# metatensor/metatrain

Hardware: AMD Instinct MI355X
Metric: atom-steps/sec (energy+forces) PET 10k-atom box (higher is better)
Workload: dtype f32; 1 GPU; PET forward + dE/dR (preprocess+features+predict+backward), 8 x 10000-atom boxes per GPU per step, default PET hypers (2.9M params), 4.5 A cutoff, 191050 edges/box; parallelism=boxes sharded over 1 rank(s), no data-path collective

## Files before the change

metatrain_amd/csrc/rows_s.h:

```cpp
#pragma once
#include "ablk.h"

namespace pet {

constexpr int RING_NW = 4;
constexpr size_t RING_LDS_BYTES = RING_NW * 16384 + RING_NSLOT * RING_SLOT;

#define RING_WAVE(R)                                                                              \
    extern __shared__ __attribute__((aligned(16))) char ring_smem[];                             \
    const RowLane L;                                                                              \
    const unsigned lane16 = (unsigned)L.lane * 16u;                                               \
    const int wave = __builtin_amdgcn_readfirstlane(threadIdx.x >> 6);                            \
    int64_t row0 = ((int64_t)blockIdx.x * RING_NW + wave) * WROWS;                                \
    const bool live = row0 < (R);                                                                 \
    if (!live) row0 = (((R) - 1) / WROWS) * WROWS;                                                \
    [[maybe_unused]] const int64_t row = row0 + L.r < (R) ? row0 + L.r : (R) - 1;                 \
    [[maybe_unused]] const bool valid = live && row0 + L.r < (R);                                 \
    char* tile = ring_smem + wave * 16384;                                                        \
    const char* ring = ring_smem + RING_NW * 16384;                                               \
    const unsigned tile_u = __builtin_amdgcn_readfirstlane((unsigned)(uintptr_t)tile);            \
    const unsigned ring_u = __builtin_amdgcn_readfirstlane((unsigned)(uintptr_t)ring)
#define RING_SLOT_DST(ring_u, wave, g) ((ring_u) + (unsigned)((g) & (RING_NSLOT - 1)) * RING_SLOT + (wave) * 1024)
#define RING_SLOT_PTR(ring, g, lane16) ((ring) + ((g) & (RING_NSLOT - 1)) * RING_SLOT + (lane16))
__device__ __forceinline__ int ring_clamp(int g, int n) { return g < n ? g : n - 1; }
template <int SPC, int NC>
__device__ __forceinline__ void ring_clamp_chunk(int& hc, int& s) {
    if (s >= SPC) { s -= SPC; hc += 1; }
    if (hc >= NC) { hc = NC - 1; s = SPC - 1; }
}

template <int EXTRA = 0>
__device__ __forceinline__ void ring_stage_sync(bool extra_in_flight = false, bool drain = false) {
    if (extra_in_flight && drain) asm volatile("s_waitcnt vmcnt(0) lgkmcnt(0)" ::: "memory");
    else if (extra_in_flight) asm volatile("s_waitcnt vmcnt(%0) lgkmcnt(0)" ::"n"(2 + EXTRA) : "memory");
    else asm volatile("s_waitcnt vmcnt(2) lgkmcnt(0)" ::: "memory");
#ifndef AB_ABL_NOBAR
    __syncthreads();
#endif
}

__device__ __forceinline__ void ring_stage_mfma(const char* slot, f32x16& a0, const f16x8& x0h, const f16x8& x0l, f32x16& a1,
                                                const f16x8& x1h, const f16x8& x1l) {
    const f16x8 w0h = *reinterpret_cast<const f16x8*>(slot);
    const f16x8 w0l = *reinterpret_cast<const f16x8*>(slot + 1024);
    AB_MFMA3(a0, w0h, w0l, x0h, x0l);
    const f16x8 w1h = *reinterpret_cast<const f16x8*>(slot + 2048);
    const f16x8 w1l = *reinterpret_cast<const f16x8*>(slot + 3072);
    AB_MFMA3(a1, w1h, w1l, x1h, x1l);
}

template <int LEAD = 0, int NT = 4, int KB = 8, class Req>
__device__ __forceinline__ void hs_gemm_r(f32x16 (&acc)[NT], const f16x8 (&xh)[KB], const f16x8 (&xl)[KB], int g0, Req req,
                                          const char* ring, unsigned lane16, bool lead = false) {
#pragma unroll
    for (int r = 0; r < (NT / 2) * KB; r++) {
        const int g = g0 + r, tp = r / KB, kb = r % KB;
        if (r < 3 && lead) ring_stage_sync<LEAD>(true);
        else ring_stage_sync();
        req(g + 3);
        ring_stage_mfma(RING_SLOT_PTR(ring, g, lane16), acc[2 * tp], xh[kb], xl[kb], acc[2 * tp + 1], xh[kb], xl[kb]);
    }
}
template <int KB>
__device__ __forceinline__ void hs_planes(const float4 (&x)[2 * KB], f16x8 (&xh)[KB], f16x8 (&xl)[KB], float f = ABS) {
#pragma unroll
    for (int kb = 0; kb < KB; kb++) {
        const float v8[8] = {x[2 * kb].x * f, x[2 * kb].y * f, x[2 * kb].z * f, x[2 * kb].w * f,
                             x[2 * kb + 1].x * f, x[2 * kb + 1].y * f, x[2 * kb + 1].z * f, x[2 * kb + 1].w * f};
        ab_split8(v8, xh[kb], xl[kb]);
    }
}
__device__ __forceinline__ float hs_vec(const float* __restrict__ v, int t, int j, int i, int h) {
    const float lo = v[32 * t + 8 * j + i], hi = v[32 * t + 8 * j + 4 + i];
    return h ? hi : lo;
}
__device__ __forceinline__ float hs_vec_s(const float* __restrict__ v, int t, int j, int i, int h) {
    const float lo = ab_sload(v + 32 * t + 8 * j + i), hi = ab_sload(v + 32 * t + 8 * j + 4 + i);
    return h ? hi : lo;
}
template <int NT>
__device__ __forceinline__ void hs_acc_rows(float4 (&y)[4 * NT], const f32x16* acc, float f, const float* __restrict__ bias = nullptr,
                                            int off = 0, int h = 0) {
#pragma unroll
    for (int t = 0; t < NT; t++)
#pragma unroll
        for (int j = 0; j < 4; j++) {
            const f32x16& a = acc[t];
            y[4 * t + j] = make_float4(a[4 * j] * f, a[4 * j + 1] * f, a[4 * j + 2] * f, a[4 * j + 3] * f);
            if (bias) {
                y[4 * t + j].x += hs_vec(bias + off, t, j, 0, h); y[4 * t + j].y += hs_vec(bias + off, t, j, 1, h);
                y[4 * t + j].z += hs_vec(bias + off, t, j, 2, h); y[4 * t + j].w += hs_vec(bias + off, t, j, 3, h);
            }
        }
}

__device__ __forceinline__ void ring_dma_rows(const float* __restrict__ X, int64_t r0, int64_t R, int ld, unsigned lds_base,
                                              const RowLane& L) {
    const float* base = X + r0 * ld;
    const int rmax = (int)(R - 1 - r0 < 31 ? R - 1 - r0 : 31);
    const int hi = L.lane >> 5, c = L.lane & 31;
#pragma unroll
    for (int j = 0; j < 16; j++) {
        const int r = 2 * j + hi, rr = r < rmax ? r : rmax;
        const unsigned off = ((unsigned)rr * (unsigned)ld + 4u * (unsigned)(c ^ (r & 15))) * 4u;
        unsigned keep;
        asm volatile("s_mov_b32 %0, m0\n\ts_mov_b32 m0, %3\n\ts_nop 0\n\tglobal_load_lds_dwordx4 %1, %2\n\ts_mov_b32 m0, %0"
                     : "=&s"(keep) : "v"(off), "s"(base), "s"(lds_base + j * 1024) : "memory");
    }
}

inline W2 lin_planes(const void* planes, const Lin& l) { return w2_planes(planes, l.n_out / 32, l.k_in / 16); }
template <class... P, class... A>
inline void launch_ring(void (*kern)(P...), int64_t rows, hipStream_t st, A... args) {
    allow_big_lds(kern, RING_LDS_BYTES);
    kern<<<cdiv(rows, RING_NW * WROWS), 256, RING_LDS_BYTES, st>>>(static_cast<P>(args)...);
}

}
```

metatrain_amd/csrc/so_rows_s.hip:

```cpp
#include "rows_s.h"
#include "tile.h"

namespace pet {

__device__ __forceinline__ float rs_pick(const float* __restrict__ v, int i, int h) { return h ? v[i + 4] : v[i]; }

__global__ __launch_bounds__(256, 2) void k_rowgemm_s(const float* __restrict__ X, int ldx, int nk, const float* __restrict__ cs,
                                                     W2 w, const float* __restrict__ bias, float* __restrict__ Y, int ldy, int nn,
                                                     int64_t R, const float* __restrict__ A ) {
    RING_WAVE(R);
    const int kbt = 8 * nk, np = nk * nn;
    const f16x8* plane = (wave & 1) ? w.l : w.h;
    auto piece = [=](int nb, int ks, int s, int g) {
        const unsigned dst = RING_SLOT_DST(ring_u, wave, g);
        ab_dma_piece(plane, (4 * nb + 2 * (s >> 3) + (wave >> 1)) * kbt + 8 * ks + (s & 7), lane16, dst);
    };
    ring_dma_rows(X, row0, R, ldx, tile_u, L);
    piece(0, 0, 0, 0);
    piece(0, 0, 1, 1);
    piece(0, 0, 2, 2);
    asm volatile("s_waitcnt vmcnt(3)" ::: "memory");
    f16x8 xh[8], xl[8];
    f32x16 acc[4];
    float scale = 0.f, inv = 0.f;
#pragma unroll 1
    for (int p = 0; p < np; p++) {
        const int nb = __builtin_amdgcn_readfirstlane(p / nk), ks = __builtin_amdgcn_readfirstlane(p - nb * nk);
        bool lead = nk == 1 && nb > 0;
        RowLane Lp = L;
        asm volatile("" : "+v"(Lp.lane), "+v"(Lp.r), "+v"(Lp.h));
        int64_t r0 = row0;
        asm volatile("" : "+s"(r0));
        if (ks == 0) {
#pragma unroll
            for (int t = 0; t < 4; t++) acc[t] = ab_zero();
        }
        if (nk > 1 || p == 0) {
            float4 x[16];
            tile128_to_frag(x, tile, Lp);
            if (cs) {
                const float* v = cs + 128 * ks;
#pragma unroll
                for (int kg = 0; kg < 16; kg++) {
                    x[kg].x *= rs_pick(v, 8 * kg + 0, Lp.h);
                    x[kg].y *= rs_pick(v, 8 * kg + 1, Lp.h);
                    x[kg].z *= rs_pick(v, 8 * kg + 2, Lp.h);
                    x[kg].w *= rs_pick(v, 8 * kg + 3, Lp.h);
                }
            }
            float sc;
            const float iv = row_pow2<16>(x, sc);
            const bool shrink = ks == 0 || sc < scale;
            const float sc_eff = shrink ? sc : scale;
            if (ks > 0) {
                const float f = sc_eff * inv;
#pragma unroll
                for (int t = 0; t < 4; t++)
#pragma unroll
                    for (int i = 0; i < 16; i++) acc[t][i] *= f;
            }
            scale = sc_eff;
            inv = shrink ? iv : inv;
#pragma unroll
            for (int kg = 0; kg < 16; kg++) { x[kg].x *= sc_eff; x[kg].y *= sc_eff; x[kg].z *= sc_eff; x[kg].w *= sc_eff; }
            hs_planes(x, xh, xl);
        }
        if (ks + 1 < nk) {
            asm volatile("s_waitcnt lgkmcnt(0)" ::: "memory");
            __builtin_amdgcn_wave_barrier();
            ring_dma_rows(X + 128 * (ks + 1), r0, R, ldx, tile_u, Lp);
            lead = true;
        }
        {
            const bool last = p + 1 == np;
            const int ksn = ks + 1 < nk ? ks + 1 : 0, nbn = ks + 1 < nk ? nb : nb + 1;
            hs_gemm_r<16>(acc, xh, xl, 0, [=](int s) {
                if (s < 16) piece(nb, ks, s, s);
                else if (last) piece(nb, ks, 15, s);
                else piece(nbn, ksn, s - 16, s);
            }, ring, lane16, lead);
        }
        if (ks + 1 < nk) continue;
        const float f = inv * ABQ_INV;
        const float* bv = bias ? bias + 128 * nb : nullptr;
#pragma unroll
        for (int g = 0; g < 2; g++) {
            float4 y[8];
#pragma unroll
            for (int t = 0; t < 2; t++)
#pragma unroll
                for (int j = 0; j < 4; j++) {
                    const f32x16& a = acc[2 * g + t];
                    y[4 * t + j] = make_float4(a[4 * j] * f, a[4 * j + 1] * f, a[4 * j + 2] * f, a[4 * j + 3] * f);
                }
            if (bv) {
                const float* v = bv + 64 * g;
#pragma unroll
                for (int kg = 0; kg < 8; kg++) {
                    y[kg].x += rs_pick(v, 8 * kg + 0, Lp.h);
                    y[kg].y += rs_pick(v, 8 * kg + 1, Lp.h);
                    y[kg].z += rs_pick(v, 8 * kg + 2, Lp.h);
                    y[kg].w += rs_pick(v, 8 * kg + 3, Lp.h);
                }
            }
            const int col = 128 * nb + 64 * g;
            int64_t r0 = row0;
            asm volatile("" : "+s"(r0));
            auto out = [&](int r) { return live && r0 + r < R ? Y + (r0 + r) * ldy + col : nullptr; };
            __builtin_amdgcn_wave_barrier();
            if (A) {
                float4 old[8];
                request_rows_addend<8>(old, Lp, [&](int r) { return A + (r0 + r < R ? r0 + r : R - 1) * ldy + col; });
                store_rows_lines_add<8>(y, old, reinterpret_cast<float*>(tile), Lp, out);
            } else
                store_rows_lines<8>(y, reinterpret_cast<float*>(tile), Lp, out);
        }
        if (nk > 1 && nb + 1 < nn) {
            asm volatile("s_waitcnt lgkmcnt(0)" ::: "memory");
            __builtin_amdgcn_wave_barrier();
            int64_t r1 = row0;
            asm volatile("" : "+s"(r1));
            ring_dma_rows(X, r1, R, ldx, tile_u, Lp);
            asm volatile("s_waitcnt vmcnt(0)" ::: "memory");
        }
    }
}


#define RS_SETUP() \
    RING_WAVE(R);  \
    const f16x8* plane = (wave & 1) ? w.l : w.h
#define RS_LANE(Lx)                            \
    RowLane Lx = L;                            \
    asm volatile("" : "+v"(Lx.lane));          \
    Lx.r = Lx.lane & 31;                       \
    Lx.h = Lx.lane >> 5
#define RS_ROW0(rx) int64_t rx = row0; asm volatile("" : "+s"(rx))

__device__ __forceinline__ void rs_store_block(const f32x16 (&acc)[4], float f, const float* __restrict__ bv, const float* __restrict__ A,
                                               float* __restrict__ Y, int ldy, int col, int64_t r0, int64_t R, bool live, char* tile,
                                               const RowLane& Lq) {
    const int64_t row = r0 + Lq.r < R ? r0 + Lq.r : R - 1;
#pragma unroll
    for (int t = 0; t < 4; t++) {
        float4 y[4];
#pragma unroll
        for (int j = 0; j < 4; j++) y[j] = make_float4(acc[t][4 * j] * f, acc[t][4 * j + 1] * f, acc[t][4 * j + 2] * f, acc[t][4 * j + 3] * f);
        if (bv) {
#pragma unroll
            for (int j = 0; j < 4; j++) {
                const float4 b4 = *reinterpret_cast<const float4*>(bv + 32 * t + 8 * j + 4 * Lq.h);
                y[j].x += b4.x; y[j].y += b4.y; y[j].z += b4.z; y[j].w += b4.w;
            }
        }
        if (A) {
            float4 a4[4];
            load_rowfrag<4>(a4, A + col + 32 * t, row, ldy, Lq.h);
#pragma unroll
            for (int j = 0; j < 4; j++) { y[j].x += a4[j].x; y[j].y += a4[j].y; y[j].z += a4[j].z; y[j].w += a4[j].w; }
        }
        __builtin_amdgcn_wave_barrier();
        store_tile32_lines(y, reinterpret_cast<float*>(tile), Y + col + 32 * t, r0, live ? R : 0, ldy, Lq);
    }
}

__device__ __forceinline__ void rs_store_block_swiglu_bwd(const f32x16 (&acc)[4], float f, const float* __restrict__ VG,
                                                          float* __restrict__ dVG, int hid, int col, int64_t r0, int64_t R, bool live,
                                                          char* tile, const RowLane& Lq) {
    const int64_t row = r0 + Lq.r < R ? r0 + Lq.r : R - 1;
#pragma unroll
    for (int t = 0; t < 4; t++) {
        float4 v4[4], g4[4], dv[4], dg[4];
        load_rowfrag<4>(v4, VG + col + 32 * t, row, 2 * hid, Lq.h);
        load_rowfrag<4>(g4, VG + hid + col + 32 * t, row, 2 * hid, Lq.h);
#pragma unroll
        for (int j = 0; j < 4; j++) {
            const float du[4] = {acc[t][4 * j] * f, acc[t][4 * j + 1] * f, acc[t][4 * j + 2] * f, acc[t][4 * j + 3] * f};
            const float sx = sigmoidf_(g4[j].x), sy = sigmoidf_(g4[j].y), sz = sigmoidf_(g4[j].z), sw = sigmoidf_(g4[j].w);
            dv[j] = make_float4(du[0] * sx, du[1] * sy, du[2] * sz, du[3] * sw);
            dg[j] = make_float4(du[0] * v4[j].x * sx * (1.f - sx), du[1] * v4[j].y * sy * (1.f - sy), du[2] * v4[j].z * sz * (1.f - sz),
                                du[3] * v4[j].w * sw * (1.f - sw));
        }
        __builtin_amdgcn_wave_barrier();
        store_tile32_lines(dv, reinterpret_cast<float*>(tile), dVG + col + 32 * t, r0, live ? R : 0, 2 * hid, Lq);
        store_tile32_lines(dg, reinterpret_cast<float*>(tile), dVG + hid + col + 32 * t, r0, live ? R : 0, 2 * hid, Lq);
    }
}
__device__ __forceinline__ void rs_store_norm_bwd(f32x16 (&a0)[4], f32x16 (&a1)[4], float f, const float* __restrict__ x,
                                                  const float* __restrict__ gamma, int ln, const float* __restrict__ dres,
                                                  float* __restrict__ out, int64_t r0, int64_t R, bool live, char* tile,
                                                  const RowLane& Lq) {
    const int64_t row = r0 + Lq.r < R ? r0 + Lq.r : R - 1;
    float s1 = 0.f, s2 = 0.f, sx = 0.f, sxx = 0.f;
#pragma unroll
    for (int b = 0; b < 2; b++)
#pragma unroll
        for (int t = 0; t < 4; t++) {
            f32x16& a = b ? a1[t] : a0[t];
            float4 x4[4];
            load_rowfrag<4>(x4, x + 128 * b + 32 * t, row, 256, Lq.h);
#pragma unroll
            for (int j = 0; j < 4; j++) {
                const float4 g = *reinterpret_cast<const float4*>(gamma + 128 * b + 32 * t + 8 * j + 4 * Lq.h);
                const float xv[4] = {x4[j].x, x4[j].y, x4[j].z, x4[j].w}, gv[4] = {g.x, g.y, g.z, g.w};
#pragma unroll
                for (int i = 0; i < 4; i++) {
                    const float d = a[4 * j + i] * f * gv[i];
                    a[4 * j + i] = d;
                    s1 += d; s2 = fmaf(d, xv[i], s2); sx += xv[i]; sxx = fmaf(xv[i], xv[i], sxx);
                }
            }
        }
    s1 = row_sum(s1); s2 = row_sum(s2); sx = row_sum(sx); sxx = row_sum(sxx);
    const float mean = ln ? sx * (1.0f / 256.0f) : 0.f;
    const float var = sxx * (1.0f / 256.0f) - mean * mean;
    const float rstd = rsqrtf(var + (ln ? 1e-5f : 1.1920928955078125e-07f));
    const float m1 = ln ? s1 * (1.0f / 256.0f) : 0.f;
    const float m2 = (s2 - mean * s1) * rstd * (1.0f / 256.0f);
#pragma unroll
    for (int b = 0; b < 2; b++)
#pragma unroll
        for (int t = 0; t < 4; t++) {
            const f32x16& a = b ? a1[t] : a0[t];
            float4 x4[4], r4[4], y[4];
            load_rowfrag<4>(x4, x + 128 * b + 32 * t, row, 256, Lq.h);
            load_rowfrag<4>(r4, dres + 128 * b + 32 * t, row, 256, Lq.h);
#pragma unroll
            for (int j = 0; j < 4; j++)
                y[j] = make_float4(r4[j].x + rstd * (a[4 * j] - m1 - (x4[j].x - mean) * rstd * m2),
                                   r4[j].y + rstd * (a[4 * j + 1] - m1 - (x4[j].y - mean) * rstd * m2),
                                   r4[j].z + rstd * (a[4 * j + 2] - m1 - (x4[j].z - mean) * rstd * m2),
                                   r4[j].w + rstd * (a[4 * j + 3] - m1 - (x4[j].w - mean) * rstd * m2));
            __builtin_amdgcn_wave_barrier();
            store_tile32_lines(y, reinterpret_cast<float*>(tile), out + 128 * b + 32 * t, r0, live ? R : 0, 256, Lq);
        }
}

template <int NORM, int EPI = 0>
__global__ __launch_bounds__(256, 2) void k_rowgemm_s_k2(const float* __restrict__ X, int ldx, const float* __restrict__ cs,
                                                        const float* __restrict__ cb, W2 w, const float* __restrict__ bias,
                                                        const float* __restrict__ A, float* __restrict__ Y, int ldy, int nn, int64_t R) {
    RS_SETUP();
    const bool full = live && row0 + WROWS <= R;
    constexpr int nk = 2, kbt = 16;
    auto piece = [=](int nb, int ks, int s, int g) {
        const unsigned dst = RING_SLOT_DST(ring_u, wave, g);
        ab_dma_piece(plane, (4 * nb + 2 * (s >> 3) + (wave >> 1)) * kbt + 8 * ks + (s & 7), lane16, dst);
    };
    ring_dma_rows(X, row0, R, ldx, tile_u, L);
    asm volatile("s_waitcnt vmcnt(0)" ::: "memory");
    f16x8 xh[2][8], xl[2][8];
    float inv;
    {
        float4 x0[16], x1[16];
        tile128_to_frag(x0, tile, L);
        asm volatile("s_waitcnt lgkmcnt(0)" ::: "memory");
        __builtin_amdgcn_wave_barrier();
        ring_dma_rows(X + 128, row0, R, ldx, tile_u, L);
        asm volatile("s_waitcnt vmcnt(0)" ::: "memory");
        tile128_to_frag(x1, tile, L);
        if (NORM) {
            float mean = 0.f;
            if (NORM == 2) {
                float s1 = 0.f;
#pragma unroll
                for (int k = 0; k < 16; k++) s1 += (x0[k].x + x0[k].y) + (x0[k].z + x0[k].w) + (x1[k].x + x1[k].y) + (x1[k].z + x1[k].w);
                mean = row_sum(s1) * (1.0f / 256.0f);
            }
            float s2 = 0.f;
#pragma unroll
            for (int k = 0; k < 16; k++) {
                if (NORM == 2) {
                    x0[k].x -= mean; x0[k].y -= mean; x0[k].z -= mean; x0[k].w -= mean;
                    x1[k].x -= mean; x1[k].y -= mean; x1[k].z -= mean; x1[k].w -= mean;
                }
                s2 += x0[k].x * x0[k].x + x0[k].y * x0[k].y + x0[k].z * x0[k].z + x0[k].w * x0[k].w;
                s2 += x1[k].x * x1[k].x + x1[k].y * x1[k].y + x1[k].z * x1[k].z + x1[k].w * x1[k].w;
            }
            const float rstd = rsqrtf(row_sum(s2) * (1.0f / 256.0f) + (NORM == 2 ? 1e-5f : 1.1920928955078125e-07f));
#pragma unroll
            for (int k = 0; k < 16; k++) {
                const float4 g0 = *reinterpret_cast<const float4*>(cs + 8 * k + 4 * L.h);
                const float4 g1 = *reinterpret_cast<const float4*>(cs + 128 + 8 * k + 4 * L.h);
                x0[k] = make_float4(x0[k].x * rstd * g0.x, x0[k].y * rstd * g0.y, x0[k].z * rstd * g0.z, x0[k].w * rstd * g0.w);
                x1[k] = make_float4(x1[k].x * rstd * g1.x, x1[k].y * rstd * g1.y, x1[k].z * rstd * g1.z, x1[k].w * rstd * g1.w);
                if (NORM == 2) {
                    const float4 b0 = *reinterpret_cast<const float4*>(cb + 8 * k + 4 * L.h);
                    const float4 b1 = *reinterpret_cast<const float4*>(cb + 128 + 8 * k + 4 * L.h);
                    x0[k].x += b0.x; x0[k].y += b0.y; x0[k].z += b0.z; x0[k].w += b0.w;
                    x1[k].x += b1.x; x1[k].y += b1.y; x1[k].z += b1.z; x1[k].w += b1.w;
                }
            }
        } else if (cs) {
#pragma unroll
            for (int k = 0; k < 16; k++) {
                const float4 g0 = *reinterpret_cast<const float4*>(cs + 8 * k + 4 * L.h);
                const float4 g1 = *reinterpret_cast<const float4*>(cs + 128 + 8 * k + 4 * L.h);
                x0[k].x *= g0.x; x0[k].y *= g0.y; x0[k].z *= g0.z; x0[k].w *= g0.w;
                x1[k].x *= g1.x; x1[k].y *= g1.y; x1[k].z *= g1.z; x1[k].w *= g1.w;
            }
        }
        float sc0, sc1;
        const float iv0 = row_pow2<16>(x0, sc0), iv1 = row_pow2<16>(x1, sc1);
        const float sc = sc0 < sc1 ? sc0 : sc1;
        inv = sc0 < sc1 ? iv0 : iv1;
#pragma unroll
        for (int k = 0; k < 16; k++) { x0[k].x *= sc; x0[k].y *= sc; x0[k].z *= sc; x0[k].w *= sc; }
        hs_planes(x0, xh[0], xl[0]);
#pragma unroll
        for (int k = 0; k < 16; k++) { x1[k].x *= sc; x1[k].y *= sc; x1[k].z *= sc; x1[k].w *= sc; }
        hs_planes(x1, xh[1], xl[1]);
    }
    asm volatile("s_waitcnt vmcnt(0) lgkmcnt(0)" ::: "memory");
    piece(0, 0, 0, 0);
    piece(0, 0, 1, 1);
    piece(0, 0, 2, 2);
    const float f = inv * ABQ_INV;
#pragma unroll 1
    for (int nb = 0; nb < nn; nb++) {
        f32x16 acc[4];
#pragma unroll
        for (int t = 0; t < 4; t++) acc[t] = ab_zero();
        const bool last = nb + 1 == nn;
        if (nb > 0 && !full) asm volatile("s_waitcnt vmcnt(0)" ::: "memory");
        if (EPI == 1 && nb > 0) asm volatile("s_waitcnt vmcnt(0)" ::: "memory");
        hs_gemm_r<16>(acc, xh[0], xl[0], 0, [=](int s) {
            if (s < 16) piece(nb, 0, s, s); else piece(nb, 1, s - 16, s);
        }, ring, lane16, EPI == 0 && nb > 0 && full);
        hs_gemm_r(acc, xh[1], xl[1], 0, [=](int s) {
            if (s < 16) piece(nb, 1, s, s);
            else if (last) piece(nb, 1, 15, s);
            else piece(nb + 1, 0, s - 16, s);
        }, ring, lane16);
        RS_LANE(Lq);
        RS_ROW0(r0);
        if (EPI == 1) rs_store_block_swiglu_bwd(acc, f, A, Y, 128 * nn, 128 * nb, r0, R, live, tile, Lq);
        else rs_store_block(acc, f, bias ? bias + 128 * nb : nullptr, A, Y, ldy, 128 * nb, r0, R, live, tile, Lq);
    }
}

template <int EPI = 0>
__global__ __launch_bounds__(256, 2) void k_rowgemm_s_n2(const float* __restrict__ X, int ldx, int nk, W2 w,
                                                        const float* __restrict__ bias, const float* __restrict__ A,
                                                        float* __restrict__ Y, int ldy, int64_t R,
                                                        const float* __restrict__ xn = nullptr, int ln = 0) {
    RS_SETUP();
    const int kbt = 8 * nk;
    auto piece = [=](int nb, int ks, int s, int g) {
        const unsigned dst = RING_SLOT_DST(ring_u, wave, g);
        ab_dma_piece(plane, (4 * nb + 2 * (s >> 3) + (wave >> 1)) * kbt + 8 * ks + (s & 7), lane16, dst);
    };
    ring_dma_rows(X, row0, R, ldx, tile_u, L);
    piece(0, 0, 0, 0);
    piece(0, 0, 1, 1);
    piece(0, 0, 2, 2);
    asm volatile("s_waitcnt vmcnt(3)" ::: "memory");
    f32x16 acc0[4], acc1[4];
#pragma unroll
    for (int t = 0; t < 4; t++) { acc0[t] = ab_zero(); acc1[t] = ab_zero(); }
    f16x8 xh[8], xl[8];
    float scale = 0.f, inv = 0.f;
#pragma unroll 1
    for (int ks = 0; ks < nk; ks++) {
        RS_LANE(Lp);
        RS_ROW0(r0);
        {
            const char* rowp = tile + 512 * Lp.r;
            const int sw = Lp.r & 15;
            float m = 0.f;
#pragma unroll
            for (int kg = 0; kg < 16; kg++) {
                const float4 v = *reinterpret_cast<const float4*>(rowp + 16 * ((2 * kg + Lp.h) ^ sw));
                m = fmaxf(fmaxf(m, fmaxf(fabsf(v.x), fabsf(v.y))), fmaxf(fabsf(v.z), fabsf(v.w)));
            }
            m = fmaxf(m, __shfl_xor(m, 32));
            int e = (__float_as_int(m) >> 23) & 0xff;
            e = e > 253 ? 253 : e;
            const float sc = __int_as_float((254 - e) << 23), iv = __int_as_float(e << 23);
            const bool shrink = ks == 0 || sc < scale;
            const float sc_eff = shrink ? sc : scale;
            if (ks > 0) {
                const float g = sc_eff * inv;
#pragma unroll
                for (int t = 0; t < 4; t++)
#pragma unroll
                    for (int i = 0; i < 16; i++) { acc0[t][i] *= g; acc1[t][i] *= g; }
            }
            scale = sc_eff;
            inv = shrink ? iv : inv;
            const float fs = sc_eff;
#pragma unroll
            for (int kb = 0; kb < 8; kb++) {
                const float4 a = *reinterpret_cast<const float4*>(rowp + 16 * ((4 * kb + Lp.h) ^ sw));
                const float4 b = *reinterpret_cast<const float4*>(rowp + 16 * ((4 * kb + 2 + Lp.h) ^ sw));
                const float v8[8] = {a.x * fs * ABS, a.y * fs * ABS, a.z * fs * ABS, a.w * fs * ABS,
                                     b.x * fs * ABS, b.y * fs * ABS, b.z * fs * ABS, b.w * fs * ABS};
                ab_split8(v8, xh[kb], xl[kb]);
            }
        }
        const bool more = ks + 1 < nk;
        if (more) {
            asm volatile("s_waitcnt lgkmcnt(0)" ::: "memory");
            __builtin_amdgcn_wave_barrier();
            ring_dma_rows(X + 128 * (ks + 1), r0, R, ldx, tile_u, Lp);
        }
        hs_gemm_r<16>(acc0, xh, xl, 0, [=](int s) {
            if (s < 16) piece(0, ks, s, s); else piece(1, ks, s - 16, s);
        }, ring, lane16, more);
        hs_gemm_r(acc1, xh, xl, 0, [=](int s) {
            if (s < 16) piece(1, ks, s, s);
            else if (!more) piece(1, ks, 15, s);
            else piece(0, ks + 1, s - 16, s);
        }, ring, lane16);
    }
    const float f = inv * ABQ_INV;
    RS_LANE(Lq);
    RS_ROW0(r0);
    asm volatile("s_waitcnt lgkmcnt(0)" ::: "memory");
    __builtin_amdgcn_wave_barrier();
    if (EPI == 1) {
        rs_store_norm_bwd(acc0, acc1, f, xn, bias, ln, A, Y, r0, R, live, tile, Lq);
        return;
    }
    rs_store_block(acc0, f, bias, A, Y, ldy, 0, r0, R, live, tile, Lq);
    rs_store_block(acc1, f, bias ? bias + 128 : nullptr, A, Y, ldy, 128, r0, R, live, tile, Lq);
}

bool rowgemm_s_ex(hipStream_t st, const float* X, int K, const float* cs, const void* planes, const float* bias, const float* A,
                  float* Y, int n_out, int64_t R, int norm, const float* cb) {
    if (!planes || K % 128 || n_out % 128 || K > 1024 || n_out > 1024 || !ring_serves(R)) return false;
    if (norm && (K != 256 || !cs || (norm == 2 && !cb))) return false;
    const W2 w = w2_planes(planes, n_out / 32, K / 16);
    if (norm == 1) launch_ring(k_rowgemm_s_k2<1>, R, st, X, K, cs, cb, w, bias, A, Y, n_out, n_out / 128, R);
    else if (norm == 2) launch_ring(k_rowgemm_s_k2<2>, R, st, X, K, cs, cb, w, bias, A, Y, n_out, n_out / 128, R);
    else if (K == 256 && n_out >= 256) launch_ring(k_rowgemm_s_k2<0>, R, st, X, K, cs, nullptr, w, bias, A, Y, n_out, n_out / 128, R);
    else if (n_out == 256 && K >= 256 && !cs) launch_ring(k_rowgemm_s_n2<0>, R, st, X, K, K / 128, w, bias, A, Y, n_out, R, nullptr, 0);
    else launch_ring(k_rowgemm_s, R, st, X, K, K / 128, cs, w, bias, Y, n_out, n_out / 128, R, A);
    return true;
}
bool rowgemm_s_swiglu_bwd(hipStream_t st, const float* X, const void* planes, const float* VG, float* dVG, int hid, int64_t R) {
    if (!planes || hid % 128 || hid > 1024 || !ring_serves(R)) return false;
    launch_ring(k_rowgemm_s_k2<0, 1>, R, st, X, 256, nullptr, nullptr, w2_planes(planes, hid / 32, 256 / 16), nullptr, VG, dVG, 2 * hid,
                hid / 128, R);
    return true;
}
bool rowgemm_s_norm_bwd(hipStream_t st, const float* X, int K, const void* planes, const float* xn, const float* gamma, int ln,
                        const float* dres, float* out, int64_t R) {
    if (!planes || K % 128 || K < 256 || K > 1024 || !ring_serves(R)) return false;
    launch_ring(k_rowgemm_s_n2<1>, R, st, X, K, K / 128, w2_planes(planes, 256 / 32, K / 16), gamma, dres, out, 256, R, xn, ln);
    return true;
}
bool rowgemm_s(hipStream_t st, const float* X, int K, const float* cs, const void* planes, const float* bias, float* Y, int n_out,
               int64_t R, bool acc) {
    return rowgemm_s_ex(st, X, K, cs, planes, bias, acc ? Y : nullptr, Y, n_out, R, 0, nullptr);
}

}
```

Measured before the change: 1.947 million atom-steps/s.

## Prefetch epilogue operands during GEMM tail stages in ring row-GEMM kernels

Adds a tail-aware GEMM loop that issues the first epilogue operand loads (residual, gate values, normalized input) during the last ring stages, with deeper vmcnt waits so the loads overlap MFMA work. The epilogues for residual add, SwiGLU backward and norm backward are restructured into software-pipelined loops that prefetch the next 32-column fragment while storing the current one. SwiGLU backward gets a new kernel variant that parks the high-half input planes in LDS to free registers. This adds register and LDS pressure and more complex waitcnt accounting, which could hurt occupancy or correctness if the counts are off.

Measured after the change: 1.930 million atom-steps/s. Within noise of the previous version (-0.9%).

```diff
diff --git a/metatrain_amd/csrc/rows_s.h b/metatrain_amd/csrc/rows_s.h
--- a/metatrain_amd/csrc/rows_s.h
+++ b/metatrain_amd/csrc/rows_s.h
@@ -61,6 +61,23 @@
         ring_stage_mfma(RING_SLOT_PTR(ring, g, lane16), acc[2 * tp], xh[kb], xl[kb], acc[2 * tp + 1], xh[kb], xl[kb]);
     }
 }
+template <int TAIL, int LEAD = 0, bool XH_LDS = false, int NT = 4, int KB = 8, class Req, class Pre>
+__device__ __forceinline__ void hs_gemm_rt(f32x16 (&acc)[NT], const f16x8 (&xh)[KB], const f16x8 (&xl)[KB], int g0, Req req, Pre pre,
+                                           const char* ring, unsigned lane16, bool lead, bool tail, const char* xh_lds = nullptr) {
+    constexpr int NS = (NT / 2) * KB;
+    static_assert(NS >= 7, "the lead's three stages and the tail's three do not overlap");
+#pragma unroll
+    for (int r = 0; r < NS; r++) {
+        const int g = g0 + r, tp = r / KB, kb = r % KB;
+        if (r == NS - 4 && tail) pre();
+        if (r < 3 && lead) ring_stage_sync<LEAD>(true);
+        else if (r >= NS - 4 && r < NS - 1 && tail) ring_stage_sync<TAIL>(true);
+        else ring_stage_sync();
+        req(g + 3);
+        const f16x8 xhk = XH_LDS ? *reinterpret_cast<const f16x8*>(xh_lds + 1024 * kb) : xh[kb];
+        ring_stage_mfma(RING_SLOT_PTR(ring, g, lane16), acc[2 * tp], xhk, xl[kb], acc[2 * tp + 1], xhk, xl[kb]);
+    }
+}
 template <int KB>
 __device__ __forceinline__ void hs_planes(const float4 (&x)[2 * KB], f16x8 (&xh)[KB], f16x8 (&xl)[KB], float f = ABS) {
 #pragma unroll
@@ -77,6 +94,10 @@
 __device__ __forceinline__ float hs_vec_s(const float* __restrict__ v, int t, int j, int i, int h) {
     const float lo = ab_sload(v + 32 * t + 8 * j + i), hi = ab_sload(v + 32 * t + 8 * j + 4 + i);
     return h ? hi : lo;
+}
+__device__ __forceinline__ float4 hs_vec4_s(const float* __restrict__ v, int kg, int h) {
+    return make_float4(hs_vec_s(v + 8 * kg, 0, 0, 0, h), hs_vec_s(v + 8 * kg, 0, 0, 1, h), hs_vec_s(v + 8 * kg, 0, 0, 2, h),
+                       hs_vec_s(v + 8 * kg, 0, 0, 3, h));
 }
 template <int NT>
 __device__ __forceinline__ void hs_acc_rows(float4 (&y)[4 * NT], const f32x16* acc, float f, const float* __restrict__ bias = nullptr,
diff --git a/metatrain_amd/csrc/so_rows_s.hip b/metatrain_amd/csrc/so_rows_s.hip
--- a/metatrain_amd/csrc/so_rows_s.hip
+++ b/metatrain_amd/csrc/so_rows_s.hip
@@ -136,8 +136,60 @@
     Lx.r = Lx.lane & 31;                       \
     Lx.h = Lx.lane >> 5
 #define RS_ROW0(rx) int64_t rx = row0; asm volatile("" : "+s"(rx))
-
+typedef const float __attribute__((address_space(1)))* rs_gptr;
+#define RS_OPAQUE_PTR(px, p)                 \
+    uintptr_t px##_bits = (uintptr_t)(p);    \
+    asm volatile("" : "+s"(px##_bits));      \
+    const rs_gptr px = (rs_gptr)px##_bits
+__device__ __forceinline__ void rs_load_rowfrag4(float4 (&x)[4], rs_gptr X, int64_t row, int ld, int h) {
+    typedef float f32x4 __attribute__((ext_vector_type(4)));
+    typedef const f32x4 __attribute__((address_space(1)))* gptr4;
+    const gptr4 p = (gptr4)(X + row * ld + 4 * h);
+#pragma unroll
+    for (int kg = 0; kg < 4; kg++) {
+        const f32x4 v = p[2 * kg];
+        x[kg] = make_float4(v.x, v.y, v.z, v.w);
+    }
+}
+
+constexpr int RS_TAIL_ADD = 4;
+constexpr int RS_TAIL_VG = 4;
+constexpr int RS_TAIL_NORM = 4;
+__device__ __forceinline__ int64_t rs_row(int64_t r0, int64_t R, const RowLane& Lq) { return r0 + Lq.r < R ? r0 + Lq.r : R - 1; }
+
+template <bool ADD, bool DEEP, bool MORE = false>
 __device__ __forceinline__ void rs_store_block(const f32x16 (&acc)[4], float f, const float* __restrict__ bv, const float* __restrict__ A,
+                                               float4 (&a0)[4], float* __restrict__ Y, int ldy, int col, int64_t r0, int64_t R, bool live,
+                                               char* tile, const RowLane& Lq) {
+    const int64_t row = rs_row(r0, R, Lq);
+#pragma unroll
+    for (int t = 0; t < 4; t++) {
+        float4 y[4], nx[4];
+        if (DEEP && ADD && (t < 3 || MORE)) load_rowfrag<4>(nx, A + col + 32 * (t + 1), row, ldy, Lq.h);
+#pragma unroll
+        for (int j = 0; j < 4; j++) y[j] = make_float4(acc[t][4 * j] * f, acc[t][4 * j + 1] * f, acc[t][4 * j + 2] * f, acc[t][4 * j + 3] * f);
+        if (bv) {
+#pragma unroll
+            for (int j = 0; j < 4; j++) {
+                const float4 b4 = hs_vec4_s(bv + 32 * t, j, Lq.h);
+                y[j].x += b4.x; y[j].y += b4.y; y[j].z += b4.z; y[j].w += b4.w;
+            }
+        }
+        if (ADD) {
+#pragma unroll
+            for (int j = 0; j < 4; j++) { y[j].x += a0[j].x; y[j].y += a0[j].y; y[j].z += a0[j].z; y[j].w += a0[j].w; }
+        }
+        if (!DEEP && ADD && (t < 3 || MORE)) load_rowfrag<4>(a0, A + col + 32 * (t + 1), row, ldy, Lq.h);
+        __builtin_amdgcn_wave_barrier();
+        store_tile32_lines(y, reinterpret_cast<float*>(tile), Y + col + 32 * t, r0, live ? R : 0, ldy, Lq);
+        if (DEEP && ADD && (t < 3 || MORE)) {
+#pragma unroll
+            for (int j = 0; j < 4; j++) a0[j] = nx[j];
+        }
+    }
+}
+
+__device__ __forceinline__ void rs_store_block_v(const f32x16 (&acc)[4], float f, const float* __restrict__ bv, const float* __restrict__ A,
                                                float* __restrict__ Y, int ldy, int col, int64_t r0, int64_t R, bool live, char* tile,
                                                const RowLane& Lq) {
     const int64_t row = r0 + Lq.r < R ? r0 + Lq.r : R - 1;
@@ -164,53 +216,85 @@
     }
 }
 
+__device__ __forceinline__ void rs_tile32_put(const float4 (&y)[4], float* lds, const RowLane& L) {
+    float* wr = lds + L.r * TILE32_LD + 4 * L.h;
+#pragma unroll
+    for (int q = 0; q < 4; q++) *reinterpret_cast<float4*>(wr + 8 * q) = y[q];
+    __builtin_amdgcn_wave_barrier();
+}
+__device__ __forceinline__ void rs_tile32_lines(const float* lds, float* __restrict__ Y, int64_t row0, int64_t n_rows, int ld,
+                                                const RowLane& L) {
+    const int rr = L.lane >> 3, cc = 4 * (L.lane & 7);
+#pragma unroll
+    for (int j = 0; j < 4; j++) {
+        const int r = 8 * j + rr;
+        const float4 v = *reinterpret_cast<const float4*>(lds + r * TILE32_LD + cc);
+        if (row0 + r < n_rows) *reinterpret_cast<float4*>(Y + (row0 + r) * ld + cc) = v;
+    }
+    __builtin_amdgcn_wave_barrier();
+}
+
 __device__ __forceinline__ void rs_store_block_swiglu_bwd(const f32x16 (&acc)[4], float f, const float* __restrict__ VG,
-                                                          float* __restrict__ dVG, int hid, int col, int64_t r0, int64_t R, bool live,
-                                                          char* tile, const RowLane& Lq) {
-    const int64_t row = r0 + Lq.r < R ? r0 + Lq.r : R - 1;
+                                                          float4 (&g4)[4], float* __restrict__ dVG, int hid, int col, int64_t r0,
+                                                          int64_t R, bool live, char* tile, const RowLane& Lq) {
+    const int64_t row = rs_row(r0, R, Lq);
+    float* lds = reinterpret_cast<float*>(tile);
 #pragma unroll
     for (int t = 0; t < 4; t++) {
-        float4 v4[4], g4[4], dv[4], dg[4];
-        load_rowfrag<4>(v4, VG + col + 32 * t, row, 2 * hid, Lq.h);
-        load_rowfrag<4>(g4, VG + hid + col + 32 * t, row, 2 * hid, Lq.h);
+        float4 v4[4], s4[4], dv[4], dg[4];
 #pragma unroll
         for (int j = 0; j < 4; j++) {
             const float du[4] = {acc[t][4 * j] * f, acc[t][4 * j + 1] * f, acc[t][4 * j + 2] * f, acc[t][4 * j + 3] * f};
             const float sx = sigmoidf_(g4[j].x), sy = sigmoidf_(g4[j].y), sz = sigmoidf_(g4[j].z), sw = sigmoidf_(g4[j].w);
+            s4[j] = make_float4(sx, sy, sz, sw);
             dv[j] = make_float4(du[0] * sx, du[1] * sy, du[2] * sz, du[3] * sw);
+        }
+        __builtin_amdgcn_wave_barrier();
+        rs_tile32_put(dv, lds, Lq);
+        load_rowfrag<4>(v4, VG + col + 32 * t, row, 2 * hid, Lq.h);
+        rs_tile32_lines(lds, dVG + col + 32 * t, r0, live ? R : 0, 2 * hid, Lq);
+#pragma unroll
+        for (int j = 0; j < 4; j++) {
+            const float du[4] = {acc[t][4 * j] * f, acc[t][4 * j + 1] * f, acc[t][4 * j + 2] * f, acc[t][4 * j + 3] * f};
+            const float sx = s4[j].x, sy = s4[j].y, sz = s4[j].z, sw = s4[j].w;
             dg[j] = make_float4(du[0] * v4[j].x * sx * (1.f - sx), du[1] * v4[j].y * sy * (1.f - sy), du[2] * v4[j].z * sz * (1.f - sz),
                                 du[3] * v4[j].w * sw * (1.f - sw));
         }
-        __builtin_amdgcn_wave_barrier();
-        store_tile32_lines(dv, reinterpret_cast<float*>(tile), dVG + col + 32 * t, r0, live ? R : 0, 2 * hid, Lq);
-        store_tile32_lines(dg, reinterpret_cast<float*>(tile), dVG + hid + col + 32 * t, r0, live ? R : 0, 2 * hid, Lq);
+        rs_tile32_put(dg, lds, Lq);
+        if (t < 3) load_rowfrag<4>(g4, VG + hid + col + 32 * (t + 1), row, 2 * hid, Lq.h);
+        rs_tile32_lines(lds, dVG + hid + col + 32 * t, r0, live ? R : 0, 2 * hid, Lq);
     }
 }
 __device__ __forceinline__ void rs_store_norm_bwd(f32x16 (&a0)[4], f32x16 (&a1)[4], float f, const float* __restrict__ x,
-                                                  const float* __restrict__ gamma, int ln, const float* __restrict__ dres,
+                                                  float4 (&x4)[4], const float* __restrict__ gamma, int ln, const float* __restrict__ dres,
                                                   float* __restrict__ out, int64_t r0, int64_t R, bool live, char* tile,
                                                   const RowLane& Lq) {
-    const int64_t row = r0 + Lq.r < R ? r0 + Lq.r : R - 1;
+    const int64_t row = rs_row(r0, R, Lq);
     float s1 = 0.f, s2 = 0.f, sx = 0.f, sxx = 0.f;
-#pragma unroll
-    for (int b = 0; b < 2; b++)
-#pragma unroll
-        for (int t = 0; t < 4; t++) {
-            f32x16& a = b ? a1[t] : a0[t];
-            float4 x4[4];
-            load_rowfrag<4>(x4, x + 128 * b + 32 * t, row, 256, Lq.h);
-#pragma unroll
-            for (int j = 0; j < 4; j++) {
-                const float4 g = *reinterpret_cast<const float4*>(gamma + 128 * b + 32 * t + 8 * j + 4 * Lq.h);
-                const float xv[4] = {x4[j].x, x4[j].y, x4[j].z, x4[j].w}, gv[4] = {g.x, g.y, g.z, g.w};
-#pragma unroll
-                for (int i = 0; i < 4; i++) {
-                    const float d = a[4 * j + i] * f * gv[i];
-                    a[4 * j + i] = d;
-                    s1 += d; s2 = fmaf(d, xv[i], s2); sx += xv[i]; sxx = fmaf(xv[i], xv[i], sxx);
-                }
-            }
-        }
+    float4 r4[4];
+#pragma unroll
+    for (int q = 0; q < 8; q++) {
+        f32x16& a = q >= 4 ? a1[q - 4] : a0[q];
+        float4 nx[4];
+        if (q < 7) load_rowfrag<4>(nx, x + 32 * (q + 1), row, 256, Lq.h);
+        else {
+            load_rowfrag<4>(nx, x, row, 256, Lq.h);
+            load_rowfrag<4>(r4, dres, row, 256, Lq.h);
+        }
+#pragma unroll
+        for (int j = 0; j < 4; j++) {
+            const float4 g = hs_vec4_s(gamma + 32 * q, j, Lq.h);
+            const float xv[4] = {x4[j].x, x4[j].y, x4[j].z, x4[j].w}, gv[4] = {g.x, g.y, g.z, g.w};
+#pragma unroll
+            for (int i = 0; i < 4; i++) {
+                const float d = a[4 * j + i] * f * gv[i];
+                a[4 * j + i] = d;
+                s1 += d; s2 = fmaf(d, xv[i], s2); sx += xv[i]; sxx = fmaf(xv[i], xv[i], sxx);
+            }
+        }
+#pragma unroll
+        for (int j = 0; j < 4; j++) x4[j] = nx[j];
+    }
     s1 = row_sum(s1); s2 = row_sum(s2); sx = row_sum(sx); sxx = row_sum(sxx);
     const float mean = ln ? sx * (1.0f / 256.0f) : 0.f;
     const float var = sxx * (1.0f / 256.0f) - mean * mean;
@@ -218,25 +302,29 @@
     const float m1 = ln ? s1 * (1.0f / 256.0f) : 0.f;
     const float m2 = (s2 - mean * s1) * rstd * (1.0f / 256.0f);
 #pragma unroll
-    for (int b = 0; b < 2; b++)
-#pragma unroll
-        for (int t = 0; t < 4; t++) {
-            const f32x16& a = b ? a1[t] : a0[t];
-            float4 x4[4], r4[4], y[4];
-            load_rowfrag<4>(x4, x + 128 * b + 32 * t, row, 256, Lq.h);
-            load_rowfrag<4>(r4, dres + 128 * b + 32 * t, row, 256, Lq.h);
-#pragma unroll
-            for (int j = 0; j < 4; j++)
-                y[j] = make_float4(r4[j].x + rstd * (a[4 * j] - m1 - (x4[j].x - mean) * rstd * m2),
-                                   r4[j].y + rstd * (a[4 * j + 1] - m1 - (x4[j].y - mean) * rstd * m2),
-                                   r4[j].z + rstd * (a[4 * j + 2] - m1 - (x4[j].z - mean) * rstd * m2),
-                                   r4[j].w + rstd * (a[4 * j + 3] - m1 - (x4[j].w - mean) * rstd * m2));
-            __builtin_amdgcn_wave_barrier();
-            store_tile32_lines(y, reinterpret_cast<float*>(tile), out + 128 * b + 32 * t, r0, live ? R : 0, 256, Lq);
-        }
-}
-
-template <int NORM, int EPI = 0>
+    for (int q = 0; q < 8; q++) {
+        const f32x16& a = q >= 4 ? a1[q - 4] : a0[q];
+        float4 y[4], nx[4], nr[4];
+        if (q < 7) {
+            load_rowfrag<4>(nx, x + 32 * (q + 1), row, 256, Lq.h);
+            load_rowfrag<4>(nr, dres + 32 * (q + 1), row, 256, Lq.h);
+        }
+#pragma unroll
+        for (int j = 0; j < 4; j++)
+            y[j] = make_float4(r4[j].x + rstd * (a[4 * j] - m1 - (x4[j].x - mean) * rstd * m2),
+                               r4[j].y + rstd * (a[4 * j + 1] - m1 - (x4[j].y - mean) * rstd * m2),
+                               r4[j].z + rstd * (a[4 * j + 2] - m1 - (x4[j].z - mean) * rstd * m2),
+                               r4[j].w + rstd * (a[4 * j + 3] - m1 - (x4[j].w - mean) * rstd * m2));
+        __builtin_amdgcn_wave_barrier();
+        store_tile32_lines(y, reinterpret_cast<float*>(tile), out + 32 * q, r0, live ? R : 0, 256, Lq);
+        if (q < 7) {
+#pragma unroll
+            for (int j = 0; j < 4; j++) { x4[j] = nx[j]; r4[j] = nr[j]; }
+        }
+    }
+}
+
+template <int NORM>
 __global__ __launch_bounds__(256, 2) void k_rowgemm_s_k2(const float* __restrict__ X, int ldx, const float* __restrict__ cs,
                                                         const float* __restrict__ cb, W2 w, const float* __restrict__ bias,
                                                         const float* __restrict__ A, float* __restrict__ Y, int ldy, int nn, int64_t R) {
@@ -323,10 +411,9 @@
         for (int t = 0; t < 4; t++) acc[t] = ab_zero();
         const bool last = nb + 1 == nn;
         if (nb > 0 && !full) asm volatile("s_waitcnt vmcnt(0)" ::: "memory");
-        if (EPI == 1 && nb > 0) asm volatile("s_waitcnt vmcnt(0)" ::: "memory");
         hs_gemm_r<16>(acc, xh[0], xl[0], 0, [=](int s) {
             if (s < 16) piece(nb, 0, s, s); else piece(nb, 1, s - 16, s);
-        }, ring, lane16, EPI == 0 && nb > 0 && full);
+        }, ring, lane16, nb > 0 && full);
         hs_gemm_r(acc, xh[1], xl[1], 0, [=](int s) {
             if (s < 16) piece(nb, 1, s, s);
             else if (last) piece(nb, 1, 15, s);
@@ -334,12 +421,136 @@
         }, ring, lane16);
         RS_LANE(Lq);
         RS_ROW0(r0);
-        if (EPI == 1) rs_store_block_swiglu_bwd(acc, f, A, Y, 128 * nn, 128 * nb, r0, R, live, tile, Lq);
-        else rs_store_block(acc, f, bias ? bias + 128 * nb : nullptr, A, Y, ldy, 128 * nb, r0, R, live, tile, Lq);
-    }
-}
-
-template <int EPI = 0>
+        rs_store_block_v(acc, f, bias ? bias + 128 * nb : nullptr, A, Y, ldy, 128 * nb, r0, R, live, tile, Lq);
+    }
+}
+
+template <int NORM, int EPI = 0, bool ADD = false>
+__global__ __launch_bounds__(256, 2) void k_rowgemm_s_k2e(const float* __restrict__ X, int ldx, const float* __restrict__ cs,
+                                                        const float* __restrict__ cb, W2 w, const float* __restrict__ bias,
+                                                        const float* __restrict__ A, float* __restrict__ Y, int ldy, int nn, int64_t R) {
+    RS_SETUP();
+    const bool full = live && row0 + WROWS <= R;
+    constexpr int nk = 2, kbt = 16;
+    constexpr bool PARK = EPI == 1;
+    constexpr int RS_PARK_OFF = 8192;
+    static_assert(32 * TILE32_LD * 4 <= RS_PARK_OFF && RS_PARK_OFF + 8 * 1024 <= 16384, "staging area, parked planes: one 16-KB tile");
+    auto piece = [=](int nb, int ks, int s, int g) {
+        const unsigned dst = RING_SLOT_DST(ring_u, wave, g);
+        ab_dma_piece(plane, (4 * nb + 2 * (s >> 3) + (wave >> 1)) * kbt + 8 * ks + (s & 7), lane16, dst);
+    };
+    ring_dma_rows(X, row0, R, ldx, tile_u, L);
+    f16x8 xh[2][8], xl[2][8];
+    float inv;
+    {
+        float4 x0[16], x1[16];
+        load_rowfrag<16>(x1, X + 128, row, ldx, L.h);
+        piece(0, 0, 0, 0);
+        piece(0, 0, 1, 1);
+        piece(0, 0, 2, 2);
+        asm volatile("s_waitcnt vmcnt(3)" ::: "memory");
+        tile128_to_frag(x0, tile, L);
+        if (NORM) {
+            float mean = 0.f;
+            if (NORM == 2) {
+                float s1 = 0.f;
+#pragma unroll
+                for (int k = 0; k < 16; k++) s1 += (x0[k].x + x0[k].y) + (x0[k].z + x0[k].w) + (x1[k].x + x1[k].y) + (x1[k].z + x1[k].w);
+                mean = row_sum(s1) * (1.0f / 256.0f);
+            }
+            float s2 = 0.f;
+#pragma unroll
+            for (int k = 0; k < 16; k++) {
+                if (NORM == 2) {
+                    x0[k].x -= mean; x0[k].y -= mean; x0[k].z -= mean; x0[k].w -= mean;
+                    x1[k].x -= mean; x1[k].y -= mean; x1[k].z -= mean; x1[k].w -= mean;
+                    s2 += x0[k].x * x0[k].x + x0[k].y * x0[k].y + x0[k].z * x0[k].z + x0[k].w * x0[k].w;
+                    s2 += x1[k].x * x1[k].x + x1[k].y * x1[k].y + x1[k].z * x1[k].z + x1[k].w * x1[k].w;
+                } else {
+#pragma clang fp contract(off)
+                    float q0, q1;
+                    if (k >= 11) {
+                        q0 = __builtin_fmaf(x0[k].w, x0[k].w, __builtin_fmaf(x0[k].z, x0[k].z, __builtin_fmaf(x0[k].x, x0[k].x, x0[k].y * x0[k].y)));
+                        q1 = __builtin_fmaf(x1[k].w, x1[k].w, __builtin_fmaf(x1[k].z, x1[k].z, __builtin_fmaf(x1[k].x, x1[k].x, x1[k].y * x1[k].y)));
+                    } else {
+                        q0 = x0[k].x * x0[k].x + x0[k].y * x0[k].y + x0[k].z * x0[k].z + x0[k].w * x0[k].w;
+                        q1 = x1[k].x * x1[k].x + x1[k].y * x1[k].y + x1[k].z * x1[k].z + x1[k].w * x1[k].w;
+                    }
+                    s2 += q0;
+                    s2 += q1;
+                }
+            }
+            const float rstd = rsqrtf(row_sum(s2) * (1.0f / 256.0f) + (NORM == 2 ? 1e-5f : 1.1920928955078125e-07f));
+#pragma unroll
+            for (int k = 0; k < 16; k++) {
+                const float4 g0 = hs_vec4_s(cs, k, L.h);
+                const float4 g1 = hs_vec4_s(cs + 128, k, L.h);
+                x0[k] = make_float4(x0[k].x * rstd * g0.x, x0[k].y * rstd * g0.y, x0[k].z * rstd * g0.z, x0[k].w * rstd * g0.w);
+                x1[k] = make_float4(x1[k].x * rstd * g1.x, x1[k].y * rstd * g1.y, x1[k].z * rstd * g1.z, x1[k].w * rstd * g1.w);
+                if (NORM == 2) {
+                    const float4 b0 = hs_vec4_s(cb, k, L.h);
+                    const float4 b1 = hs_vec4_s(cb + 128, k, L.h);
+                    x0[k].x += b0.x; x0[k].y += b0.y; x0[k].z += b0.z; x0[k].w += b0.w;
+                    x1[k].x += b1.x; x1[k].y += b1.y; x1[k].z += b1.z; x1[k].w += b1.w;
+                }
+            }
+        } else if (cs) {
+#pragma unroll
+            for (int k = 0; k < 16; k++) {
+                const float4 g0 = hs_vec4_s(cs, k, L.h);
+                const float4 g1 = hs_vec4_s(cs + 128, k, L.h);
+                x0[k].x *= g0.x; x0[k].y *= g0.y; x0[k].z *= g0.z; x0[k].w *= g0.w;
+                x1[k].x *= g1.x; x1[k].y *= g1.y; x1[k].z *= g1.z; x1[k].w *= g1.w;
+            }
+        }
+        float sc0, sc1;
+        const float iv0 = row_pow2<16>(x0, sc0), iv1 = row_pow2<16>(x1, sc1);
+        const float sc = sc0 < sc1 ? sc0 : sc1;
+        inv = sc0 < sc1 ? iv0 : iv1;
+#pragma unroll
+        for (int k = 0; k < 16; k++) { x0[k].x *= sc; x0[k].y *= sc; x0[k].z *= sc; x0[k].w *= sc; }
+        hs_planes(x0, xh[0], xl[0]);
+#pragma unroll
+        for (int k = 0; k < 16; k++) { x1[k].x *= sc; x1[k].y *= sc; x1[k].z *= sc; x1[k].w *= sc; }
+        hs_planes(x1, xh[1], xl[1]);
+        if (PARK) {
+#pragma unroll
+            for (int kb = 0; kb < 8; kb++) *reinterpret_cast<f16x8*>(tile + RS_PARK_OFF + 1024 * kb + lane16) = xh[1][kb];
+        }
+    }
+    const float f = inv * ABQ_INV;
+    constexpr int STORES = EPI == 1 ? 32 : 16;
+    constexpr int TAIL = EPI == 1 ? RS_TAIL_VG : RS_TAIL_ADD;
+    constexpr bool tail = EPI == 1 || ADD;
+    RS_OPAQUE_PTR(Aq, A);
+#pragma unroll 1
+    for (int nb = 0; nb < nn; nb++) {
+        f32x16 acc[4];
+#pragma unroll
+        for (int t = 0; t < 4; t++) acc[t] = ab_zero();
+        const bool last = nb + 1 == nn;
+        if (nb > 0 && !full) asm volatile("s_waitcnt vmcnt(0)" ::: "memory");
+        hs_gemm_r<STORES>(acc, xh[0], xl[0], 0, [=](int s) {
+            if (s < 16) piece(nb, 0, s, s); else piece(nb, 1, s - 16, s);
+        }, ring, lane16, nb > 0 && full);
+        RS_LANE(Lq);
+        RS_ROW0(r0);
+        float4 e0[4];
+        hs_gemm_rt<TAIL, 0, PARK>(acc, xh[1], xl[1], 0, [=](int s) {
+            if (s < 16) piece(nb, 1, s, s);
+            else if (last) piece(nb, 1, 15, s);
+            else piece(nb + 1, 0, s - 16, s);
+        }, [&]() {
+            const int64_t rw = rs_row(r0, R, Lq);
+            if (EPI == 1) rs_load_rowfrag4(e0, Aq + 128 * nn + 128 * nb, rw, 256 * nn, Lq.h);
+            else rs_load_rowfrag4(e0, Aq + 128 * nb, rw, ldy, Lq.h);
+        }, ring, lane16, false, tail, tile + RS_PARK_OFF + lane16);
+        if (EPI == 1) rs_store_block_swiglu_bwd(acc, f, A, e0, Y, 128 * nn, 128 * nb, r0, R, live, tile, Lq);
+        else rs_store_block<ADD, false>(acc, f, bias ? bias + 128 * nb : nullptr, A, e0, Y, ldy, 128 * nb, r0, R, live, tile, Lq);
+    }
+}
+
+template <int EPI = 0, bool ADD = false>
 __global__ __launch_bounds__(256, 2) void k_rowgemm_s_n2(const float* __restrict__ X, int ldx, int nk, W2 w,
                                                         const float* __restrict__ bias, const float* __restrict__ A,
                                                         float* __restrict__ Y, int ldy, int64_t R,
@@ -360,6 +571,7 @@
     for (int t = 0; t < 4; t++) { acc0[t] = ab_zero(); acc1[t] = ab_zero(); }
     f16x8 xh[8], xl[8];
     float scale = 0.f, inv = 0.f;
+    float4 e0[4];
 #pragma unroll 1
     for (int ks = 0; ks < nk; ks++) {
         RS_LANE(Lp);
@@ -407,11 +619,13 @@
         hs_gemm_r<16>(acc0, xh, xl, 0, [=](int s) {
             if (s < 16) piece(0, ks, s, s); else piece(1, ks, s - 16, s);
         }, ring, lane16, more);
-        hs_gemm_r(acc1, xh, xl, 0, [=](int s) {
+        RS_OPAQUE_PTR(Eq, EPI == 1 ? xn : A);
+        hs_gemm_rt<EPI == 1 ? RS_TAIL_NORM : RS_TAIL_ADD>(acc1, xh, xl, 0, [=](int s) {
             if (s < 16) piece(1, ks, s, s);
             else if (!more) piece(1, ks, 15, s);
             else piece(0, ks + 1, s - 16, s);
-        }, ring, lane16);
+        }, [&]() { rs_load_rowfrag4(e0, Eq, rs_row(r0, R, Lp), EPI == 1 ? 256 : ldy, Lp.h); },
+        ring, lane16, false, EPI == 1 || ADD);
     }
     const float f = inv * ABQ_INV;
     RS_LANE(Lq);
@@ -419,11 +633,11 @@
     asm volatile("s_waitcnt lgkmcnt(0)" ::: "memory");
     __builtin_amdgcn_wave_barrier();
     if (EPI == 1) {
-        rs_store_norm_bwd(acc0, acc1, f, xn, bias, ln, A, Y, r0, R, live, tile, Lq);
+        rs_store_norm_bwd(acc0, acc1, f, xn, e0, bias, ln, A, Y, r0, R, live, tile, Lq);
         return;
     }
-    rs_store_block(acc0, f, bias, A, Y, ldy, 0, r0, R, live, tile, Lq);
-    rs_store_block(acc1, f, bias ? bias + 128 : nullptr, A, Y, ldy, 128, r0, R, live, tile, Lq);
+    rs_store_block<ADD, true, true>(acc0, f, bias, A, e0, Y, ldy, 0, r0, R, live, tile, Lq);
+    rs_store_block<ADD, true>(acc1, f, bias ? bias + 128 : nullptr, A, e0, Y, ldy, 128, r0, R, live, tile, Lq);
 }
 
 bool rowgemm_s_ex(hipStream_t st, const float* X, int K, const float* cs, const void* planes, const float* bias, const float* A,
@@ -434,13 +648,14 @@
     if (norm == 1) launch_ring(k_rowgemm_s_k2<1>, R, st, X, K, cs, cb, w, bias, A, Y, n_out, n_out / 128, R);
     else if (norm == 2) launch_ring(k_rowgemm_s_k2<2>, R, st, X, K, cs, cb, w, bias, A, Y, n_out, n_out / 128, R);
     else if (K == 256 && n_out >= 256) launch_ring(k_rowgemm_s_k2<0>, R, st, X, K, cs, nullptr, w, bias, A, Y, n_out, n_out / 128, R);
+    else if (n_out == 256 && K >= 256 && !cs && A) launch_ring(k_rowgemm_s_n2<0, true>, R, st, X, K, K / 128, w, bias, A, Y, n_out, R, nullptr, 0);
     else if (n_out == 256 && K >= 256 && !cs) launch_ring(k_rowgemm_s_n2<0>, R, st, X, K, K / 128, w, bias, A, Y, n_out, R, nullptr, 0);
     else launch_ring(k_rowgemm_s, R, st, X, K, K / 128, cs, w, bias, Y, n_out, n_out / 128, R, A);
     return true;
 }
 bool rowgemm_s_swiglu_bwd(hipStream_t st, const float* X, const void* planes, const float* VG, float* dVG, int hid, int64_t R) {
     if (!planes || hid % 128 || hid > 1024 || !ring_serves(R)) return false;
-    launch_ring(k_rowgemm_s_k2<0, 1>, R, st, X, 256, nullptr, nullptr, w2_planes(planes, hid / 32, 256 / 16), nullptr, VG, dVG, 2 * hid,
+    launch_ring(k_rowgemm_s_k2e<0, 1>, R, st, X, 256, nullptr, nullptr, w2_planes(planes, hid / 32, 256 / 16), nullptr, VG, dVG, 2 * hid,
                 hid / 128, R);
     return true;
 }
```
